# bwohlberg/sporco

Measured on AMD Instinct MI355X. Metric: ConvBPDN ADMM iterations/s, higher is better.
Workload: dtype f32; 1 GPU; admm.cbpdn.ConvBPDN 512x512 greyscale, K=64 8x8 filters, N=32 images per GPU, lambda=0.05, default options (AutoRho, stats every iteration); global_images=32, parallelism=image-shard x1

## Files before the change

sporco_amd/csrc/api_admm_run.inc:

```
    bool admm_run_supported(const sporco_amd_admm_params &p) const {
        return !cplx && std::is_same<T, float>::value && rows_ok && mr_ok(p) && (fused || fused_slabs) && !fused_mc &&
               !tail_mode && !(p.flags & (F_XRRS | F_GRADREG | F_KEEP_X | F_FEVAL_Y)) &&
               (!(p.flags & F_JOINT) || joint_rows_ok(p)) && p.lmbda >= 0.0 && p.rho > 0.0 &&
               !std::getenv("SPORCO_AMD_HOST_LOOP");
    }

    bool persist_ok(const sporco_amd_admm_params &p, const sporco_amd_admm_ctrl &c, bool vf,
                    bool has_reduce) const {
        const bool off = sw.persist >= 0 ? sw.persist != 1 : !hint_one_launch;
        return !off && vf && !has_reduce && fused && !fused_slabs && Ks == K && run_always_emit &&
               admm_persist_supported<T>(H, W, K) && !wl1.ptr && c.max_iter >= 3 &&
               !(p.flags & (F_NOBNDRY | F_AMS | F_JOINT)) && admm_persist_resident<T>(H, W, K, CN);
    }
    PersistIterArgs<T> persist_iter_args(const sporco_amd_admm_params &p, const T *vin, T *vout,
                                         double *prow, double *pcol) {
        PersistIterArgs<T> a;
        cx<T> *Xf = cv(SPORCO_AMD_VAR_XF);
        a.fwd.y = a.fwd.u = nullptr;
        a.fwd.v = vin;
        a.fwd.flags = p.flags;
        a.fwd.C = C;
        a.fwd.N = N;
        a.fwd.dH = p.dH;
        a.fwd.dW = p.dW;
// ... 69 lines not shown
        a.iter[p0] = persist_iter_args(p, v_prev, v_other, part_rows, part_f);
        a.iter[p0 ^ 1] = persist_iter_args(p, v_other, v_prev, pst_part_rows, pst_part_f);
        a.blk = static_cast<PersistIterArgs<T> *>(pst_blk);
        a.ctl_blk = pst_ctl;
        a.ctl = ctl_dev;
        a.rec = reinterpret_cast<AdmmRecord *>(rec_ring) + index0;
        a.index0 = index0;
        a.max_iter = max_iter - index0;
        a.bar = pst_bar;
        a.n_row_tiles = (int)nrow;
        a.n_col_tiles = (int)ncol;
        a.want_dfid = (p.flags & F_OBJ) ? 1 : 0;
        a.want_sums = want_sums ? 1 : 0;
        a.dfid_scale = 1.0 / ((double)H * W);
        SA_HIP(hipMemsetAsync(pst_bar, 0, sizeof(unsigned) * kPersistBarWords, st));
        {
            ProfScope ps(prof, PS_PERSIST);
            launch_admm_persist<T>(st, a, grid);
        }
        unsigned bar[16];
        SA_HIP(hipMemcpyAsync(bar, pst_bar, sizeof(bar), hipMemcpyDeviceToHost, st));
        sync();
        if (bar[2]) throw Error(SPORCO_AMD_EHIP, "one-launch solve: a grid barrier did not complete");
        xf_tiled = true;
        ++pst_runs;
        return (int)bar[3];
    }

    int64_t enqueue_iter_ctl(const sporco_amd_admm_params &p, const T *vin = nullptr,
                             T *vout = nullptr) {
        T *Y = vin ? nullptr : static_cast<T *>(vars[SPORCO_AMD_VAR_Y]);
        T *U = vin ? nullptr : static_cast<T *>(vars[SPORCO_AMD_VAR_U]);
        cx<T> *Xf = cv(SPORCO_AMD_VAR_XF);
        {
            RowsFwdArgs<T> ra;
            ra.y = Y;
            ra.u = U;
            ra.v = vin;
            ra.flags = p.flags;
            ra.C = C;
            ra.N = N;
            if (vin) {
                ra.wl1 = wl1;
                ra.dH = p.dH;
                ra.dW = p.dW;
                ra.ams_bits = ams_bits_of(p);
                ra.ams_k = Ku - 1;
            }
            ra.s2 = T(1);
            ra.t = Xf;
            ra.Ks = Ks;
            ra.twA = twRows;
            ra.H = H;
            ra.W = W;
            ra.CN = CN;
            ra.K = K;
            ra.P = P;
            ra.ctl = ctl_dev;
            ProfScope ps(prof, vin ? PS_ROWS_FWD_V : PS_ROWS_FWD);
            launch_rows_fwd<T>(st, ra);
        }
        {
            FusedColsArgs<T> fa;
            fa.t = Xf;
            fa.dft = dft;
            fa.sft = sft;
            fa.gramt = gramt;
            fa.twA = twA;
            fa.twB = twB;
            fa.rho = (T)p.rho;
            fa.H = H;
            fa.W = W;
            fa.CN = CN;
            fa.K = K;
            fa.partials = part_f;
            fa.Ks = Ks;
            fa.ctl = ctl_dev;
            if (cols_striped() && !fused_slabs) {
                fa.out_even = cols_out[0];
                fa.out_odd = cols_out[1];
            }
            ProfScope ps(prof, PS_FUSED_COLS);
            if (fused_slabs) {
                FusedSlabArgs<T> sa;
                sa.c = fa;
                sa.qpart = qpart;
                part_f_rows = (int)run_slab_cols(sa);
            } else {
                part_f_rows = (int)launch_fused_cols<T>(st, fa);
            }
            xf_tiled = true;
        }
        RowsPostArgs<T> pa;
        pa.twA = twRows;
        pa.t_next = nullptr;
        pa.t = Xf;
        if (cols_striped() && !fused_slabs) {
            pa.t = cols_out[0];
            pa.t_odd = cols_out[1];
        }
        pa.twW = planW.tw<T>();
        pa.y = Y;
        pa.u = U;
        pa.y_out = y_alt;
        pa.u_out = u_alt;
        pa.v_in = vin;
        pa.v_out = vout;
        pa.x = nullptr;
        pa.scale = T(1.0 / ((double)H * (double)W));
        pa.rlx = (T)p.rlx;
        pa.thr = T(0);
        pa.u_scale = T(1);
        pa.flags = p.flags;
// ... 204 lines not shown
        x_stale = true;
        x_invalid = p.flags & F_NO_X;
        prev_in_alt = !vf;
        return n;
    }

    void rows_inverse_to(T *Xout, const cx<T> *t_in = nullptr) {
        RowsProxArgs<T> ra;
        ra.t_in = t_in ? t_in : cv(SPORCO_AMD_VAR_XF);
        ra.Ks = t_in ? 0 : Ks;
        ra.t_out = nullptr;
        ra.x = Xout;
        ra.twA = twRows;
        ra.twW = planW.tw<T>();
        ra.scale = T(1.0 / ((double)H * (double)W));
        ra.thr = T(0);
        ra.flags = 0;
        ra.H = H;
        ra.W = W;
        ra.C = C;
        ra.N = N;
        ra.K = K;
        ra.dH = 1;
        ra.dW = 1;
        ra.P = P;
        ra.wl1 = Weight<T>();
        ra.partials = part_rows;
        ProfScope ps(prof, PS_FFT_C2R);
        launch_rows_inv_prox_fwd<T>(st, ra);
    }

    void launch_rows_fwd_on(const T *Yin, const T *Uin, T s2, const T *Vin = nullptr,
                            T thr_prev = T(0), uint32_t flags = 0, T thr21_prev = T(0),
                            const sporco_amd_admm_params *vp = nullptr, cx<T> *t_out = nullptr) {
        RowsFwdArgs<T> ra;
        if (Vin && vp) {
            ra.wl1 = wl1;
            ra.dH = vp->dH;
            ra.dW = vp->dW;
            ra.ams_bits = ams_bits_of(*vp);
            ra.ams_k = Ku - 1;
        }
        ra.y = Yin;
        ra.u = Uin;
        ra.v = Vin;
        ra.thr_prev = thr_prev;
        ra.thr21_prev = thr21_prev;
        ra.flags = flags;
        ra.C = C;
        ra.N = N;
        ra.s2 = s2;
        ra.t = t_out ? t_out : cv(SPORCO_AMD_VAR_XF);
        ra.Ks = Ks;
        ra.twA = twRows;
        ra.H = H;
        ra.W = W;
        ra.CN = CN;
        ra.K = K;
        ra.P = P;
        ProfScope ps(prof, Vin ? PS_ROWS_FWD_V : PS_ROWS_FWD);
        launch_rows_fwd<T>(st, ra);
    }
```

sporco_amd/csrc/api_setup.inc:

```
    void set_signal(const void *S) override {
        before_state_change();
        SA_HIP(hipMemcpyAsync(sreal, S, sizeof(T) * (int64_t)H * W * CNs, hipMemcpyHostToDevice, st));
        fwd2(sreal, nullptr, T(0), cv(SPORCO_AMD_VAR_SF), CNs);
        if (cplx_pair) pm_pair(cv(SPORCO_AMD_VAR_SF), cv(SPORCO_AMD_VAR_SF), 1, N, 1);
        refresh_fused_signal();
        sync();
        have_signal = true;
    }

    void set_signal_dev(const void *S_dev) override {
        before_state_change();
        SA_HIP(hipMemcpyAsync(sreal, S_dev, sizeof(T) * (int64_t)H * W * CNs,
                              hipMemcpyDeviceToDevice, st));
        fwd2(sreal, nullptr, T(0), cv(SPORCO_AMD_VAR_SF), CNs);
        if (cplx_pair) pm_pair(cv(SPORCO_AMD_VAR_SF), cv(SPORCO_AMD_VAR_SF), 1, N, 1);
        refresh_fused_signal();
        sync();
        have_signal = true;
    }

    void set_dict(const void *D, int dH, int dW) override {
        SA_REQUIRE(dH >= 1 && dW >= 1 && dH <= H && dW <= W,
                   "filter support must fit inside the signal");
        before_dict_change();
// ... 181 lines not shown
                materialize_x();
                prev_in_alt = keep;
                ProfScope ps(prof, PS_OTHER);
                launch_relax<T>(st, rv(SPORCO_AMD_VAR_X), y_alt, rv(SPORCO_AMD_VAR_AX),
                                (T)last_p.rlx, E);
            }
        }
        before_read(var);
        host_copy(var, dst, false);
        sync();
    }
    void *device_ptr(int var) override {
        before_read(var);
        return var_ptr(var);
    }

    void read_out(const double *out_dev, double *out_host) override {
        SA_HIP(hipMemcpyAsync(out_pinned, out_dev, sizeof(double) * kOutSlots, hipMemcpyDeviceToHost,
                              st));
        sync();
        std::memcpy(out_host, out_pinned, sizeof(double) * kOutSlots);
    }

    void require_single_channel_dict() const {
        if (Cd > 1)
            throw Error(SPORCO_AMD_EINVAL,
                        "multi-channel dictionaries are handled by the ADMM ConvBPDN calls only");
    }
    void require_ready() const {
        if (!have_dict || !have_signal)
            throw Error(SPORCO_AMD_ESTATE, "set_signal and set_dict must be called first");
    }

    bool run_fused_cols(const sporco_amd_admm_params &p, double *out_dev, bool striped = false) {
        if (fused_mc) {
            SA_REQUIRE(!(p.flags & (F_GRADREG | F_AMS | F_JOINT)),
                       "this solver variant needs a single-channel dictionary");
            if (!binv_valid || binv_rho != p.rho) {
                ProfScope ps(prof, PS_OTHER);
                launch_mc_binv<T>(st, dft_mc, bt_mc, npix, Cd, K, (T)p.rho);
                binv_valid = true;
                binv_rho = p.rho;
            }
            FusedMcArgs<T> ma;
            ma.t = cv(SPORCO_AMD_VAR_XF);
            ma.dft = dft_mc;
            ma.sft = sft_mc;
            ma.bt = bt_mc;
            ma.twA = twA;
            ma.twB = twB;
            ma.rho = (T)p.rho;
            ma.H = H;
            ma.W = W;
            ma.N = N;
            ma.K = K;
            ma.Cd = Cd;
            ma.partials = part_f;
            int64_t nt;
            {
                ProfScope ps(prof, PS_FUSED_COLS);
                nt = launch_fused_cols_mc<T>(st, ma);
            }
            part_f_rows = (int)nt;
            xf_tiled = true;
            if (out_dev && (p.flags & F_OBJ) && !(p.flags & F_FEVAL_Y)) {
                const int slots[1] = {SPORCO_AMD_OUT_DFID};
                const double scales[1] = {1.0 / ((double)H * W)};
// ... 37 lines not shown
        }
        int64_t ntiles;
        bool did_stripe = false;
        if (tail_ok) {
            if (!sft_eff) {
                SA_HIP(hipMalloc((void **)&sft_eff, sizeof(cx<T>) * npix * CN));
                SA_HIP(hipMalloc((void **)&coef_t, sizeof(cx<T>) * npix * CN));
            }
            const int Kt = K - 64;
            const int64_t nt = (int64_t)Wf * CN, tstride = (int64_t)H * Ks;
            cx<T> *tail = fa.t + 64;
            fa.Kv = 64;
            fa.Ks = Ks;
            fa.coef_out = coef_t;
            ProfScope ps(prof, PS_FUSED_COLS);
            fft_c2c<T>(st, planH, false, tail, tail, nt, Kt, tstride, Ks, tstride, Ks, T(1));
            launch_tail_inner<T>(st, fa, sft, sft_eff);
            fa.sft = sft_eff;
            ntiles = launch_fused_cols<T>(st, fa);
            launch_tail_update<T>(st, fa);
            fft_c2c<T>(st, planH, true, tail, tail, nt, Kt, tstride, Ks, tstride, Ks, T(1));
        } else if (fused_slabs) {
            FusedSlabArgs<T> sa;
            sa.c = fa;
            sa.qpart = qpart;
            ProfScope ps(prof, PS_FUSED_COLS);
            ntiles = run_slab_cols(sa);
            if (gradreg) ntiles *= (K + 63) / 64;
        } else {
            striped = striped && cols_striped() && !gradreg;
            if (striped) {
                fa.out_even = cols_out[0];
                fa.out_odd = cols_out[1];
            }
            ProfScope ps(prof, PS_FUSED_COLS);
            ntiles = launch_fused_cols<T>(st, fa);
            did_stripe = striped;
        }
        part_f_rows = (int)ntiles;
        xf_tiled = true;
        if (out_dev && (p.flags & F_OBJ) && !(p.flags & F_FEVAL_Y)) {
            const int slots[2] = {SPORCO_AMD_OUT_DFID, SPORCO_AMD_OUT_RGR};
            const double scales[2] = {1.0 / ((double)H * W), 1.0 / ((double)H * W)};
            const int nv = gradreg ? 2 : 1;
            finalize(part_f, (int)ntiles, nv, nv, slots, scales, out_dev);
        }
        return did_stripe;
    }

    void admm_iter_fused(const sporco_amd_admm_params &p, double *out_dev) {
        require_ready();
        if (gv_live) ensure_yu();
        const bool keep_x = p.flags & F_KEEP_X;
        const bool nn = p.flags & F_NONNEG, jn = p.flags & F_JOINT;
        if (v_live && (!vform_ok(p) || !vform_same_opts(p))) ensure_yu();
        const bool vf = vform_ok(p) && (v_live || touch_epoch == fused_epoch);
        T *vin = vf && v_live ? v_cur : nullptr;
        if (!keep_x && !y_alt) alloc_alt_pair();
        T *Y = vin ? nullptr : rv(SPORCO_AMD_VAR_Y), *U = vin ? nullptr : rv(SPORCO_AMD_VAR_U);
        cx<T> *Xf = cv(SPORCO_AMD_VAR_XF);
        T *vout = vf ? (vin == y_alt ? u_alt : y_alt) : nullptr;
        if (!(t_ready && p.u_scale == 1.0)) {
            if (vin) launch_rows_fwd_on(nullptr, nullptr, (T)p.u_scale, vin, v_thr, p.flags, v_thr21, &p);
            else launch_rows_fwd_on(Y, U, (T)p.u_scale);
        }
        t_ready = false;
        const bool striped = run_fused_cols(p, nullptr, !keep_x);
        stable_run = p.u_scale == 1.0 ? stable_run + 1 : 0;
        const bool emit = stable_run >= 2 && !sw.no_speculation;
        RowsPostArgs<T> pa;
        pa.twA = twRows;
        pa.t_next = emit ? Xf : nullptr;
        pa.t = Xf;
        if (striped) {
            pa.t = cols_out[0];
            pa.t_odd = cols_out[1];
        }
        pa.twW = planW.tw<T>();
        pa.y = Y;
        pa.u = U;
        pa.y_out = keep_x ? Y : y_alt;
        pa.u_out = keep_x ? U : u_alt;
        pa.v_in = vin;
        pa.v_out = vout;
        pa.thr_prev = v_thr;
        pa.thr21_prev = v_thr21;
        pa.x = keep_x ? rv(SPORCO_AMD_VAR_X) : nullptr;
        pa.scale = T(1.0 / ((double)H * (double)W));
        pa.rlx = (T)p.rlx;
        pa.thr = (T)(p.lmbda / p.rho);
        pa.thr21 = (T)(p.mu / p.rho);
        pa.u_scale = (T)p.u_scale;
        pa.flags = p.flags;
        pa.H = H;
        pa.W = W;
        pa.C = C;
        pa.N = N;
        pa.K = K;
        pa.dH = p.dH;
        pa.dW = p.dW;
// ... 60 lines not shown
```

sporco_amd/csrc/csc_api.hip:

```cpp
#include "csc_impl.h"

#include <chrono>
#include <string>

namespace sporco_amd {

thread_local std::string g_last_error;
std::atomic<int64_t> g_xfer[4];
const char *kProfNames[PS_COUNT] = {"fft_r2c_rows",     "fft_c2c_cols_fwd", "sm_solve",
                                           "fft_c2c_cols_inv", "fft_c2r_rows",     "admm_post",
                                           "fused_cols_sm",    "rows_fwd",         "rows_inv_post",
                                           "rows_inv_post_emit",
                                           "rows_fwd_v",       "rows_inv_post_v",  "rows_inv_post_v_emit",
                                           "pgm_grad_ifft",    "pgm_rows_prox",    "pgm_fft_momentum",
                                           "finalize",         "pgm_elementwise",  "other",
                                           "admm_persist_run",
                                    "setcoef_rows",     "setcoef_cols",     "ccmod_grad_tiled",
                                    "fft_c2r_vpost",    "fft_c2r_vpost_emit",
                                    "inhib_update"};

struct Switches {
    bool unfused, old_rows, no_pad, no_vform, no_speculation, no_cols_sm, md_generic, cns_generic, cg_host,
        placement_off, placement_force;
    int persist;
    int cols_sm_force_slab;
    static bool set(const char *name) { return std::getenv(name) != nullptr; }
    static Switches read() {
        Switches s;
        s.unfused = set("SPORCO_AMD_UNFUSED");
        s.old_rows = set("SPORCO_AMD_OLD_ROWS");
        s.no_pad = set("SPORCO_AMD_NO_PAD");
        s.no_vform = set("SPORCO_AMD_NO_VFORM");
        s.no_speculation = set("SPORCO_AMD_NO_SPECULATION");
        s.no_cols_sm = set("SPORCO_AMD_NO_COLS_SM");
        s.md_generic = set("SPORCO_AMD_MD_GENERIC");
        s.cns_generic = set("SPORCO_AMD_CNS_GENERIC");
        s.cg_host = set("SPORCO_AMD_CG_HOST");
        const char *e = std::getenv("SPORCO_AMD_PLACEMENT");
        s.placement_off = e && e[0] == '0';
        s.placement_force = e && e[0] == 'f';
        e = std::getenv("SPORCO_AMD_PERSIST");
        s.persist = e ? (e[0] == '1' ? 1 : 0) : -1;
        e = std::getenv("SPORCO_AMD_COLS_SM_FORCE_SLAB");
        s.cols_sm_force_slab = e ? std::atoi(e) : 0;
        return s;
    }
};

template <typename T> struct Csc : CscBase {
    const Switches sw = Switches::read();
    sporco_amd_dims dm;
    int device;
    hipStream_t st = nullptr;
    bool own_stream = false;
    int H, W, Wf, C, N, K, CN;
    int Ku;
    int Cd = 1, Cs, CNs;
    cx<T> *ism_gam = nullptr, *ism_del = nullptr, *ism_mm = nullptr;
    bool fused_mc = false;
    cx<T> *dft_mc = nullptr, *sft_mc = nullptr;
    T *bt_mc = nullptr;
    bool binv_valid = false;
    double binv_rho = 0.0;
    cx<T> *cns_f = nullptr;
    static constexpr int kTailMax = 8;
    int Ks = 0;
    int64_t EFt = 0;
    bool tail_mode = false;
    cx<T> *sft_eff = nullptr, *coef_t = nullptr;
    uint32_t *ams_bits = nullptr;
    bool ams_bits_valid = false;
    T *cns_m = nullptr, *cns_yold = nullptr;
    bool cns_active = false;
// ... 227 lines not shown
    }
    void big_alloc_fresh(void **p, size_t bytes) {
        if (bytes >= ((size_t)64 << 20)) {
            const size_t al = (size_t)kAllocAlignMb << 20;
            void *base = nullptr;
            SA_HIP(hipMalloc(&base, bytes + al));
            const uintptr_t b = reinterpret_cast<uintptr_t>(base);
            *p = reinterpret_cast<void *>((b + al - 1) / al * al);
            skew_reg.emplace_back(*p, base);
            return;
        }
        SA_HIP(hipMalloc(p, bytes));
    }
    void big_free(void *p) {
        if (!p) return;
        for (auto &e : skew_reg)
            if (e.first == p) {
                (void)hipFree(e.second);
                e.first = nullptr;
                return;
            }
        (void)hipFree(p);
    }

    ~Csc() override {
        (void)hipSetDevice(device);
        (void)hipStreamSynchronize(st);
        place_release_spares();
        inhib_release();
        big_free(gemit);
        if (part_vpost) (void)hipFree(part_vpost);
        big_free(cols_out[0]);
        big_free(cols_out[1]);
        for (hipEvent_t e : place_ev)
            if (e) (void)hipEventDestroy(e);
        for (auto &v : vars) big_free(v);
        big_free(y_alt);
        big_free(u_alt);
        big_free(work);
        y_alt = u_alt = nullptr;
        work = nullptr;
        for (void *p : {(void *)pst_part_rows, (void *)pst_part_f, pst_blk, (void *)pst_ctl, (void *)pst_bar,
                        (void *)cns_w, (void *)cns_sft, (void *)flt_h, (void *)flt_w,
                        (void *)zf_ch, (void *)zfv_buf, (void *)md_sft, (void *)md_coef, (void *)pgm_rx[0], (void *)pgm_rx[1]})
            if (p) (void)hipFree(p);
        for (void *p : {(void *)dft, (void *)sft, (void *)gramt, (void *)part_f, (void *)twA, (void *)twB,
                        (void *)twRows, (void *)part_rows, (void *)y_alt, (void *)u_alt, (void *)part_pgm, (void *)part_pgm2, (void *)ccmod_r, (void *)pgm_ey, (void *)gpart,
                        (void *)qpart, (void *)coop_flags, (void *)ghh, (void *)ghw, (void *)wg, (void *)g1t, (void *)ism_gam, (void *)ism_del, (void *)ism_mm, (void *)dft_mc, (void *)sft_mc, (void *)bt_mc, (void *)cns_f, (void *)cns_m, (void *)sft_eff, (void *)coef_t, (void *)ams_bits, (void *)gramz_t,
                        (void *)cns_yold, (void *)md_s, (void *)dism_gam, (void *)dism_del, (void *)dism_mm,
                        (void *)dwork, (void *)pcn_stats, (void *)work, (void *)innerb, (void *)gram, (void *)dpad, (void *)sreal,
                        (void *)wl1_buf, (void *)wl21_buf, (void *)wams_buf, (void *)wdat_buf, (void *)part_a, (void *)part_b, (void *)part_cs, (void *)df_im, (void *)pgm_es[0], (void *)pgm_es[1], (void *)pgm_es[2], (void *)pgm_es[3],
                        (void *)out_dev_own})
            if (p) (void)hipFree(p);
        if (out_pinned) (void)hipHostFree(out_pinned);
        if (coop_err) (void)hipHostFree(coop_err);
        if (rec_ring) (void)hipHostFree(rec_ring);
        if (cg_pin) (void)hipHostFree((void *)cg_pin);
        if (cg_dev) (void)hipFree(cg_dev);
        if (ctl_dev) (void)hipFree(ctl_dev);
        planW.destroy();
        planH.destroy();
        if (depth > 1) planD.destroy();
        if (own_stream) (void)hipStreamDestroy(st);
    }

    int64_t KD() const { return (int64_t)Cd * K; }
// ... 46 lines not shown
    void sync() override {
        SA_HIP(hipStreamSynchronize(st));
        if (coop_err && *coop_err) {
            *coop_err = 0;
            throw Error(SPORCO_AMD_EHIP, "cooperating slab workgroups: a partner's partial sums never "
                                         "arrived; the iterates of this handle are invalid");
        }
    }
    bool pgm_fused_ok() const {
        return rows_ok && (cols256 || mr) && (fused || (fused_slabs && !tail_mode && !mr));
    }
    bool hint_vform = false, hint_one_launch = false;
    bool cplx_pair = false;
    void set_hint(int what, int value) override {
        if (what == SPORCO_AMD_HINT_KEEP_VFORM) hint_vform = value != 0;
        else if (what == SPORCO_AMD_HINT_ONE_LAUNCH) hint_one_launch = value != 0;
        else if (what == SPORCO_AMD_MODE_COMPLEX_PAIR) {
            SA_REQUIRE(Cd == 2 && Cs == 2, "complex pair mode: a handle with two channels (real, imaginary)");
            SA_REQUIRE(!have_signal && !zf_ch, "complex pair mode is set before the signal and the coefficient maps");
            cplx_pair = value != 0;
        } else if (what == SPORCO_AMD_VOLUME_FILTER_DEPTH) {
            SA_REQUIRE(depth > 1 && value >= 1 && value <= depth, "filter depth: a volume handle, 1 <= value <= depth");
            SA_REQUIRE(!flt_h, "volume handle: one filter support (no multi-scale dictionary)");
            vol_dD = value;
        } else throw Error(SPORCO_AMD_EINVAL, "unknown hint");
    }
    void pm_pair(const cx<T> *src, cx<T> *dst, int mid, int inner, int mode) {
        ProfScope ps(prof, PS_OTHER);
        launch_pm_butterfly<T>(st, src, dst, npix, mid, inner, W, mode);
    }
    std::string placement() override { return placement_report(); }
    cx<T> *cols_out[2] = {nullptr, nullptr};
    bool cols_striped() const { return cols_out[0] != nullptr; }
    void alloc_cols_out() {
        if (cols_out[0] || !std::is_same<T, float>::value || !fused || fused_slabs || tail_mode || Ks != K || !rows_ok || mr)
            return;
        const size_t plane = sizeof(cx<T>) * (size_t)CN * H * K;
        const size_t be = plane * (size_t)((Wf + 1) / 2), bo = plane * (size_t)(Wf / 2);
        if (!placement_on(be)) return;
        void *p0 = nullptr;
        big_alloc(&p0, be);
        cols_out[0] = static_cast<cx<T> *>(p0);
        cols_out[1] = static_cast<cx<T> *>(place_alloc(bo, {{p0, be}}, "cols_out_odd"));
    }
    void alloc_alt_pair() {
        if (y_alt) return;
        (void)var_ptr(SPORCO_AMD_VAR_XF);
        place_var(SPORCO_AMD_VAR_XF, {SPORCO_AMD_VAR_Y, SPORCO_AMD_VAR_U}, "T");
        void *t = vars[SPORCO_AMD_VAR_XF];
        const size_t tb = var_alloc_bytes(SPORCO_AMD_VAR_XF), nb = sizeof(T) * (size_t)E;
        y_alt = static_cast<T *>(place_alloc(nb, {{t, tb}}, "V0"));
        u_alt = static_cast<T *>(place_alloc(nb, {{t, tb}}, "V1"));
        place_var(SPORCO_AMD_VAR_Y, {SPORCO_AMD_VAR_XF}, "Y");
        place_var(SPORCO_AMD_VAR_U, {SPORCO_AMD_VAR_XF}, "U");
        alloc_cols_out();
        place_release_spares();
    }
    int query(int what) override {
        if (what == SPORCO_AMD_QUERY_FUSED_COLS) return (fused || fused_slabs || fused_mc) ? 1 : 0;
        if (what == SPORCO_AMD_QUERY_FUSED_ROWS) return rows_ok ? 1 : 0;
        if (what == SPORCO_AMD_QUERY_FUSED_PGM) return pgm_fused_ok() ? 1 : 0;
        if (what == SPORCO_AMD_QUERY_DEVICE_FILTERS) return K;
        if (what == SPORCO_AMD_QUERY_VFORM_LIVE) return (v_live || gv_live) ? 1 : 0;
        if (what == SPORCO_AMD_QUERY_PERSIST_RUNS) return pst_runs;
        if (what == SPORCO_AMD_QUERY_CCMOD_GROUPS) return ccmod_group_count();
        throw Error(SPORCO_AMD_EINVAL, "unknown query");
    }

#include "api_placement.inc"
#include "api_transforms.inc"
#include "api_setup.inc"
#include "api_admm_run.inc"
#include "api_admm.inc"
#include "api_pgm.inc"
#include "api_dictupdate.inc"
#include "api_consensus.inc"
// ... 13 lines not shown
```

sporco_amd/csrc/csc_fused.h:

```cpp
#pragma once

#include "common.h"
#include "csc_kernels.h"

namespace sporco_amd {

constexpr int kColsStaggerGroups = 4, kColsStaggerSleeps = 2;

template <typename E>
void launch_permute_ab(hipStream_t st, const E *in, E *out, int64_t A, int64_t B, int64_t C,
                       int64_t in_stride = 0, int64_t out_stride = 0);

template <typename T> struct FusedColsArgs {
    cx<T> *t;
    const cx<T> *dft;
    const cx<T> *sft;
    const T *gramt;
    const cx<T> *twA;
    const cx<T> *twB;
    T rho;
    int H, W, CN, K;
    double *partials;
    int Kv = 0;
    cx<T> *coef_out = nullptr;
    int Ks = 0;
    int per_tile = 0;
    int stagger_groups = 1, stagger_sleeps = 0;
    const AdmmCtl *ctl = nullptr;
    cx<T> *out_even = nullptr, *out_odd = nullptr;
    const T *g1t = nullptr;
    T *g1t_out = nullptr;
    const T *ghh = nullptr, *ghw = nullptr, *wg = nullptr;
    T mu = T(0);
};
template <typename T>
void launch_tail_inner(hipStream_t st, const FusedColsArgs<T> &a, const cx<T> *sft, cx<T> *sft_eff);
template <typename T> void launch_tail_update(hipStream_t st, const FusedColsArgs<T> &a);
template <typename T> void launch_gram_rows(hipStream_t st, const cx<T> *z, T *out, int64_t nrows, int K);
template <typename T> void launch_grad_g1(hipStream_t st, const FusedColsArgs<T> &a);

template <typename T> struct FusedSlabArgs {
    FusedColsArgs<T> c;
    cx<T> *qpart;
    unsigned *coop_flags = nullptr;
    unsigned coop_seq = 0;
    int *coop_err = nullptr;
    const cx<T> *pgm_yf = nullptr;
    T pgm_inv_L = T(0);
    cx<T> *pgm_ey = nullptr;
};
template <typename T> int64_t launch_cols_slab_coop(hipStream_t st, const FusedSlabArgs<T> &a);
template <typename T> int64_t launch_pgm_grad_slabs(hipStream_t st, const FusedSlabArgs<T> &a);
template <typename T> bool fused_slabs_supported(int H, int K);

template <typename T> struct FusedMcArgs {
    cx<T> *t;
    const cx<T> *dft;
    const cx<T> *sft;
    const T *bt;
    const cx<T> *twA, *twB;
    T rho;
    int H, W, N, K, Cd;
// ... 18 lines not shown
```

sporco_amd/csrc/csc_fused_body.inc:

```

    constexpr int H = N1 * NW;
    constexpr bool MR = mr_length(N1);
    constexpr int J = MR ? (N1 > NW ? 2 : 1) : N1 / NW;
    constexpr int LBW = ilog2(NW);
    static_assert(!MR || (NW == 16 && LP == 1), "mixed-radix heights: 16 waves, one line per group");
    constexpr int FP = LP * NW, Q = J / LP;
    static_assert(J % LP == 0, "lines per group must divide the lines per thread");
    static_assert(FP * NW * 64 <= kExchUnitsMax, "exchange group too large");
    const int tid = threadIdx.x;
    const int k = tid & 63;
    const int w = sa_readfirstlane(tid >> 6);
    const int K = (KC && !KRT) ? KC : ((KRT && a.Ks) ? a.Ks : a.K);
    const bool kv = KC == 64 ? true : k < K;
    const int xcd = blockIdx.x & 7;
    f2 *LA = dyn_lds<f2>();
    f2 *LB = LA;
    double *scratch = reinterpret_cast<double *>(LA + FP * NW * 64);
    const cf zero = mk<float>(0.f, 0.f);
    const int cvoff = k == 0 ? 0 : (int)0x80000000;
    const int ko = (w * K + k) * (int)sizeof(cf);
    int token = 0;
    if constexpr (AOFF >= 0) {
        if (a.ctl && a.ctl->stop) return;
        if constexpr (PERSIST) {
            const int ph = (int)(blockIdx.x >> 3) % a.stagger_groups;
            for (int i = 0; i < ph * a.stagger_sleeps; ++i) __builtin_amdgcn_s_sleep(127);
        }
    }
    for (int slot = blockIdx.x >> 3;; slot += gridDim.x >> 3) {
    SA_ARGS_PTR_T(FusedColsArgs<float>) ap;
    if constexpr (AOFF >= 0) ap = sa_args_reload<PERSIST, AOFF>(a);
    else ap = sa_opaque_sptr(afix);
    const int Wf = ap->W / 2 + 1, CN = ap->CN;
    if (slot >= ((Wf + 7) / 8) * CN) break;
    const int wf = (slot / CN) * 8 + xcd;
    if (wf >= Wf) break;
    const int tile = wf * CN + slot % CN;
    const AdmmCtl *ctl = ap->ctl;
    const float rho = ctl ? ctl->rho_f : ap->rho;
    const float *GH = ap->ghh + w;
    const cf *twA = ap->twA + w * N1;
    const cf *twB = ap->twB + w * (J * NW);
    const BufRsrc Tb = make_rsrc(ap->t + (int64_t)tile * H * K, (uint32_t)(H * K * sizeof(cf)));
    const int dsel = PER_TILE ? tile : wf;
    const BufRsrc Db = make_rsrc(ap->dft + (int64_t)dsel * H * K, (uint32_t)(H * K * sizeof(cf)));
    cf *const coef_out = KRT ? ap->coef_out : nullptr;
    const BufRsrc Cb = make_rsrc(coef_out ? coef_out + (int64_t)tile * H : nullptr,
                                 coef_out ? (uint32_t)(H * sizeof(cf)) : 0u);
    const cf *S = ap->sft + (int64_t)tile * H + w;
    const float *G = (GRAD ? ap->g1t : ap->gramt) + (int64_t)dsel * H + w;

    unsigned long long ts[16] = {0};
    SA_TS(0)
    cf v[N1];
#pragma unroll
    for (int h1 = 0; h1 < N1; ++h1)
        v[h1] = (kv && DBG != 2 && DBG != 4) ? buf_load_cf_x<(AOFF < 0)>(Tb, ko, NW * h1 * K * (int)sizeof(cf))
                                 : mk<float>((float)(k + h1), (float)(w - h1));
    if constexpr (DBG != 1) {
    dif1<N1, false>(v, 0);
    reg_fence<N1>(v, 0, token);
#pragma unroll
    for (int i = 1; i < N1; ++i) {
        cf tw;
        if constexpr (KC == 64 && !GRAD) sa_uload2(reinterpret_cast<const float *>(twA + i), tw.re, tw.im);
        else tw = twA[i];
        v[i] = cmul(v[i], tw);
    }
    reg_fence<N1>(v, 0, token);
    }
    SA_TS(1)

    float obj = 0.f;
    if constexpr (DBG != 1) {
    float ak = 0.f, bk = 0.f, gw = 0.f, rg = 0.f;
    if constexpr (GRAD) {
// ... 173 lines not shown
```

sporco_amd/csrc/csc_rows.h:

```cpp
#pragma once

#include "common.h"
#include "csc_fused.h"
#include "csc_kernels.h"

namespace sporco_amd {

template <typename T> struct RowsFwdArgs {
    const T *y, *u;
    T s2;
    cx<T> *t;
    const cx<T> *twA;
    int H, W, CN, K;
    int64_t P;
    const T *v = nullptr;
    T thr_prev = T(0);
    uint32_t flags = 0;
    T thr21_prev = T(0);
    int C = 1, N = 0;
    Weight<T> wl1;
    int dH = 1, dW = 1;
    const uint32_t *ams_bits = nullptr;
    int ams_k = -1;
    int y_bcast = 0;
    int Ks = 0;
    const AdmmCtl *ctl = nullptr;
    int persist = 0;
    int stagger_groups = 1, stagger_sleeps = 0;
};

template <typename T> struct RowsPostArgs {
    const cx<T> *t;
    const cx<T> *t_odd = nullptr;
    const cx<T> *twW;
    const cx<T> *twA;
    cx<T> *t_next;
    int emit_u = 0;
    const T *y, *u;
    T *y_out, *u_out;
    T *x;
    const T *v_in = nullptr;
    T *v_out = nullptr;
    T thr_prev = T(0);
    T thr21_prev = T(0);
// ... 69 lines not shown
```

sporco_amd/csrc/csc_rows_body.inc:

```
#include "csc_rows.h"

#include <cmath>
#include <cstdlib>

#include "csc_ctl_dev.h"
#include "csc_fused_body.h"
#include "regfft.h"

namespace sporco_amd {

namespace {

using namespace regfft;

struct alignas(16) cf2 {
    cf a, b;
};

constexpr int kN1 = 32;
constexpr size_t rows_lds_bytes(int NW) {
    return sizeof(f2) * 16 * NW * 64 + sizeof(double) * 8 * 16;
}

template <int N1, int NW> constexpr int spectral_waves() { return regfft::mr_length(N1) ? (N1 + 1) / 2 : NW; }
// ... 12 lines not shown

__host__ __device__ constexpr bool first_half4(int k1) {
    return k1 < 4 || k1 == 8 || (k1 >= 13 && k1 <= 19) || k1 == 24 || k1 > 28;
}
__host__ __device__ constexpr int group_of(int N1, int NW, int k1) {
    if (NW == 4) return first_half4(k1) ? 0 : 1;
    return NW == 16 ? (k1 >= (N1 + 1) / 2 ? 1 : 0) : ((k1 < 8 || k1 == 16 || k1 > 24) ? 0 : 1);
}
__host__ __device__ constexpr int kl_of(int N1, int NW, int k1) {
    if (NW == 4) {
        int r = 0;
        for (int o = 0; o < k1; ++o) r += first_half4(o) == first_half4(k1) ? 1 : 0;
        return r;
    }
    if (NW == 16) return k1 >= (N1 + 1) / 2 ? k1 - (N1 + 1) / 2 : k1;
    if (group_of(N1, NW, k1) == 0) return k1 < 8 ? k1 : (k1 == 16 ? 8 : k1 - 16);
    return k1 < 16 ? k1 - 8 : k1 - 9;
}

__device__ __forceinline__ float soft1(float v, float thr) {
    float m = fabsf(v) - thr;
    m = m > 0.f ? m : 0.f;
    return __builtin_copysignf(m, v);
}
__device__ __forceinline__ float soft1_pos(float v, float thr) { return v - sa_med3(v, -thr, thr); }
template <int MODE> __device__ __forceinline__ float soft1_m(float v, float thr) {
    if constexpr (MODE == 1) return soft1(v, thr);
    else return soft1_pos(v, thr);
}

template <int NW, bool COH = false, int N1 = kN1>
__device__ __forceinline__ void spatial_to_spectral(cf (&v)[N1], const cf *twA, cf *t, int CN, int H,
                                                    int K, int cn, int k, int h, bool pv, int w,
                                                    int lane, f2 *L, int &token) {
    constexpr int J = spectral_lines<N1, NW>(), NA = spectral_waves<N1, NW>();
    constexpr int NG = 2;
    constexpr int LPG = J / NG;
    constexpr int LBW = ilog2(NW);
    const bool act = NA >= NW || w < NA;
    dif1<N1, false>(v, 0);
#pragma unroll
    for (int i = 1; i < N1; ++i) {
        cf tw;
        sa_uload2(reinterpret_cast<const float *>(twA + w * N1 + i), tw.re, tw.im);
        v[i] = cmul(v[i], tw);
    }
    reg_fence<N1>(v, 0, token);

    cf z[J * NW];
    static_for<NG>([&](auto gc) {
        constexpr int g = decltype(gc)::value;
#pragma unroll
        for (int k1 = 0; k1 < N1; ++k1) {
            if (group_of(N1, NW, k1) != g) continue;
            const cf x = v[pos1<N1>(k1)];
            f2 t;
            t.x = x.re;
            t.y = x.im;
            L[(kl_of(N1, NW, k1) * NW + w) * 64 + lane] = t;
        }
        __syncthreads();
        if (act && (g == 0 || second_line<N1>(w))) {
#pragma unroll
            for (int jl = 0; jl < LPG; ++jl) {
                const int j = g * LPG + jl;
                const int kl = kl_of(N1, NW, line_of<N1, NW>(w, j));
#pragma unroll
                for (int n2 = 0; n2 < NW; ++n2) {
                    const f2 t = L[(kl * NW + n2) * 64 + lane];
                    z[NW * j + n2] = mk<float>(t.x, t.y);
                }
            }
        } else if (act) {
#pragma unroll
            for (int i = 0; i < LPG * NW; ++i) z[NW * g * LPG + i] = mk<float>(0.f, 0.f);
        }
        if (g + 1 < NG) __syncthreads();
    });
    if (!act) return;

#pragma unroll
    for (int j = 0; j < J; ++j) dif<NW, false>(z, NW * j);

    const int64_t tline = (int64_t)CN * H * K;
    cf *Tl = t + (int64_t)cn * H * K + (int64_t)h * K + k;
    auto store_unit = [&](int f, cf zf, cf zp) {
        cf2 ab;
        ab.a = mk<float>(0.5f * (zf.re + zp.re), 0.5f * (zf.im - zp.im));
        ab.b = mk<float>(0.5f * (zf.im + zp.im), 0.5f * (zp.re - zf.re));
        if (pv) {
            const float q[4] = {ab.a.re, ab.a.im, ab.b.re, ab.b.im};
            if constexpr (COH) sa_coh_store4(reinterpret_cast<float *>(Tl + (int64_t)f * tline), q);
            else sa_stream_store4(reinterpret_cast<float *>(Tl + (int64_t)f * tline), q);
        }
    };
#pragma unroll
    for (int pr = 0; pr < J / 2; ++pr) {
        const int ja = 2 * pr, jb = 2 * pr + 1;
        const int k1a = line_of<N1, NW>(w, ja), k1b = line_of<N1, NW>(w, jb);
        if (pr == 0 && w == 0) {
#pragma unroll
            for (int k2 = 0; k2 <= NW / 2; ++k2) {
                const cf zf = z[NW * ja + brev(k2 % NW, LBW)];
                const cf zp = z[NW * ja + brev((NW - k2) % NW, LBW)];
                store_unit(N1 * k2, zf, zp);
            }
            if constexpr ((N1 & 1) == 0) {
#pragma unroll
            for (int k2 = 0; k2 < NW / 2; ++k2) {
                const cf zf = z[NW * jb + brev(k2, LBW)];
                const cf zp = z[NW * jb + brev(NW - 1 - k2, LBW)];
                store_unit(N1 / 2 + N1 * k2, zf, zp);
            }
            }
        } else {
#pragma unroll
            for (int k2 = 0; k2 < NW / 2; ++k2) {
                store_unit(k1a + N1 * k2, z[NW * ja + brev(k2, LBW)],
                           z[NW * jb + brev(NW - 1 - k2, LBW)]);
                store_unit(k1b + N1 * k2, z[NW * jb + brev(k2, LBW)],
                           z[NW * ja + brev(NW - 1 - k2, LBW)]);
            }
        }
    }
}

// ... 214 lines not shown
                    float q0 = y0 * y0, q1 = y1 * y1;
                    sum_over_rows2(q0, q1);
                    float f0 = sa_fma(-thr21_p, sa_rsq(q0), 1.f);
                    float f1 = sa_fma(-thr21_p, sa_rsq(q1), 1.f);
                    f0 = f0 > 0.f ? f0 : 0.f;
                    f1 = f1 > 0.f ? f1 : 0.f;
                    y0 = f0 * y0;
                    y1 = f1 * y1;
                }
                y0 = sa_med3(y0, am_e[0] ? -__builtin_inff() : nn_lo, __builtin_inff());
                y1 = sa_med3(y1, am_e[1] ? -__builtin_inff() : nn_lo, __builtin_inff());
                if constexpr (GENERAL) {
                    const int n1 = half * HB + i;
                    const float keep = (hkill || NW * n1 + w >= x0kill) ? 0.f : 1.f;
                    const float mkeep = ((mbits >> n1) & 1u) ? 0.f : 1.f;
                    y0 *= am_e[0] ? mkeep : keep;
                    y1 *= am_e[1] ? mkeep : keep;
                }
                yv[i] = mk<float>(y0, y1);
                uv[i] = mk<float>(vv.re - y0, vv.im - y1);
            }
        }
#pragma unroll
        for (int i = 0; i < HB; ++i) {
#pragma clang fp contract(off)
            if (half * HB + i >= N1) continue;
            v[half * HB + i] = mk<float>(sa_fma(-s2, uv[i].re, yv[i].re), sa_fma(-s2, uv[i].im, yv[i].im));
        }
        if constexpr ((N1 & 1) == 0) reg_fence<HB>(v, half * HB, token);
        else if (half == 0) reg_fence<HB>(v, 0, token);
        else reg_fence<N1 - HB>(v, HB, token);
    }
    spatial_to_spectral<NW, COH, N1>(v, a->twA, a->t, a->CN, a->H, a->Ks ? a->Ks : a->K, cn, k, h, pv, w, lane, L,
                                     token);
}

template <typename A, typename F>
__device__ __forceinline__ void rows_tile_loop(const A &a_in, int tiles_x, int tiles_y, F &&tile_fn) {
    const int64_t ntiles = (int64_t)tiles_x * tiles_y;
    if (a_in.persist) {
        const int ph = (int)(blockIdx.x % (unsigned)a_in.stagger_groups);
        for (int i = 0; i < ph * a_in.stagger_sleeps; ++i) __builtin_amdgcn_s_sleep(127);
    }
    for (int64_t t = blockIdx.x; t < ntiles; t += gridDim.x) {
        tile_fn(sa_args_reload(a_in), (int)(t % tiles_x), (int)(t / tiles_x));
        __syncthreads();
    }
}

template <int NW, bool BCAST, bool VFORM = false, bool JOINT = false, int MODE = 0, int N1 = kN1>
__global__ void __launch_bounds__(NW * 64) rows_fwd_kernel(const RowsFwdArgs<float> a_in) {
    if (a_in.ctl && (a_in.ctl->stop | a_in.ctl->skip_fwd)) return;
    const int tiles_x = JOINT ? a_in.N * (a_in.K >> 5) : (int)((a_in.P + 127) / 128);
    rows_tile_loop(a_in, tiles_x, a_in.H,
                   [](auto a, int bx, int h) { rows_fwd_tile<NW, BCAST, VFORM, JOINT, MODE, false, N1>(a, bx, h); });
}

constexpr int batch_of(int n, int want) {
    int b = 1;
    for (int d = 1; d <= want; ++d)
        if (n % d == 0) b = d;
    return b;
}
template <int NW, bool WRITE_X, int MODE, bool EMIT_T, bool JOINT, int SF, bool COH = false, int N1 = kN1,
          typename AP>
__device__ __forceinline__ void rows_inv_post_tile(AP a, int bx, int h, int tiles_x) {
    constexpr bool GENERAL = MODE != 0;
// ... 543 lines not shown
        return 1;
    } else {
        return 2;
    }
}

template <int NW, int N1, bool EMIT, int MODE, bool JOINT>
void rows_post_variant(dim3 grid, hipStream_t st, const RowsPostArgs<float> &a) {
    if (a.v_out) {
        SA_REQUIRE(!a.x, "the V form has no X output");
        if (a.v_in) rows_launch<NW, &rows_inv_post_kernel<NW, false, MODE, EMIT, JOINT, 2, N1>>(grid, st, a);
        else rows_launch<NW, &rows_inv_post_kernel<NW, false, MODE, EMIT, JOINT, 1, N1>>(grid, st, a);
        return;
    }
    SA_REQUIRE(!a.v_in, "a V-form input needs a V-form output");
    if constexpr (!JOINT) {
        if (a.x) return rows_launch<NW, &rows_inv_post_kernel<NW, true, MODE, EMIT, false, 0, N1>>(grid, st, a);
    }
    rows_launch<NW, &rows_inv_post_kernel<NW, false, MODE, EMIT, JOINT, 0, N1>>(grid, st, a);
}
template <int NW, int N1, bool EMIT> void rows_post_emit(dim3 grid, hipStream_t st, RowsPostArgs<float> &a) {
    if (a.flags & F_JOINT) return rows_post_variant<NW, N1, EMIT, 0, true>(grid, st, a);
    const int mode = rows_mode<N1>(a);
    if (mode == 0) rows_post_variant<NW, N1, EMIT, 0, false>(grid, st, a);
    else if (mode == 1) rows_post_variant<NW, N1, EMIT, 1, false>(grid, st, a);
    else if constexpr (!mr_length(N1)) rows_post_variant<NW, N1, EMIT, 2, false>(grid, st, a);
}

}

template <int NW, int N1> void rows_fwd_launch(hipStream_t st, RowsFwdArgs<float> a) {
    constexpr bool MR = regfft::mr_length(N1);
    SA_REQUIRE(!(MR && a.y_bcast), "mixed-radix widths: no broadcast form");
    if (a.v && (a.flags & F_JOINT)) {
        SA_REQUIRE(rows_joint_supported<float>(a.W, a.C, a.K) && a.C * a.N == a.CN && !a.wl1.ptr && !a.ams_bits &&
                       !(a.flags & F_NOBNDRY),
                   "configuration not handled by the joint row pass");
        const dim3 jgrid = rows_grid(a, NW, (int64_t)a.N * (a.K / 32), a.H, 0);
        return rows_launch<NW, &rows_fwd_kernel<NW, false, true, true, 0, N1>>(jgrid, st, a);
    }
    const dim3 grid = rows_grid(a, NW, ceil_div(a.P, 128), a.H, 0);
    if (!a.v) {
        if constexpr (!MR) {
            if (a.y_bcast) return rows_launch<NW, &rows_fwd_kernel<NW, true, false, false, 0, N1>>(grid, st, a);
        }
        return rows_launch<NW, &rows_fwd_kernel<NW, false, false, false, 0, N1>>(grid, st, a);
    }
    const int mode = rows_mode<N1>(a);
    SA_REQUIRE(mode == 0 || a.C * a.N == a.CN, "the derivation needs the channel / image split");
    if (mode == 0) rows_launch<NW, &rows_fwd_kernel<NW, false, true, false, 0, N1>>(grid, st, a);
    else if (mode == 1) rows_launch<NW, &rows_fwd_kernel<NW, false, true, false, 1, N1>>(grid, st, a);
    else if constexpr (!MR) rows_launch<NW, &rows_fwd_kernel<NW, false, true, false, 2, N1>>(grid, st, a);
}

template <int NW, int N1> int64_t rows_inv_post_launch(hipStream_t st, RowsPostArgs<float> a) {
    SA_REQUIRE(!(regfft::mr_length(N1) && a.t_odd), "mixed-radix widths: no striped spectrum");
    const bool joint = a.flags & F_JOINT;
    if (joint) {
        SA_REQUIRE(!a.v_in || a.v_out, "a V-form input needs a V-form output");
        SA_REQUIRE(rows_joint_supported<float>(a.W, a.C, a.K) && !a.wl1.ptr && !a.ams_bits &&
                       !(a.flags & F_NOBNDRY) && !a.x,
                   "configuration not handled by the joint row epilogue");
    }
    const int64_t tx = joint ? (int64_t)a.N * (a.K / 32) : ceil_div(a.P, 128);
    const dim3 grid = rows_grid(a, NW, tx, a.H, a.t_next != nullptr);
    if (a.t_next) rows_post_emit<NW, N1, true>(grid, st, a);
// ... 24 lines not shown
```

Measured before the change: 390.2 iterations/s (512x512, K=64, N=32 per GPU; summed over GPUs).

## Stripe row-FFT spectrum output into even/odd buffers with separate placement

After: 390.1 iterations/s (512x512, K=64, N=32 per GPU; summed over GPUs) (median of 3 runs). About the same (-0.0%).

```diff
diff --git a/sporco_amd/csrc/api_admm_run.inc b/sporco_amd/csrc/api_admm_run.inc
--- a/sporco_amd/csrc/api_admm_run.inc
+++ b/sporco_amd/csrc/api_admm_run.inc
@@ -125,6 +125,7 @@
         T *Y = vin ? nullptr : static_cast<T *>(vars[SPORCO_AMD_VAR_Y]);
         T *U = vin ? nullptr : static_cast<T *>(vars[SPORCO_AMD_VAR_U]);
         cx<T> *Xf = cv(SPORCO_AMD_VAR_XF);
+        const bool tstripe = tfwd_striped(p);
         {
             RowsFwdArgs<T> ra;
             ra.y = Y;
@@ -142,6 +143,7 @@
             }
             ra.s2 = T(1);
             ra.t = Xf;
+            if (tstripe) ra.t_odd = tfwd_odd;
             ra.Ks = Ks;
             ra.twA = twRows;
             ra.H = H;
@@ -172,6 +174,7 @@
             if (cols_striped() && !fused_slabs) {
                 fa.out_even = cols_out[0];
                 fa.out_odd = cols_out[1];
+                if (tstripe) fa.t_odd = tfwd_odd;
             }
             ProfScope ps(prof, PS_FUSED_COLS);
             if (fused_slabs) {
@@ -442,7 +445,8 @@
 
     void launch_rows_fwd_on(const T *Yin, const T *Uin, T s2, const T *Vin = nullptr,
                             T thr_prev = T(0), uint32_t flags = 0, T thr21_prev = T(0),
-                            const sporco_amd_admm_params *vp = nullptr, cx<T> *t_out = nullptr) {
+                            const sporco_amd_admm_params *vp = nullptr, cx<T> *t_out = nullptr,
+                            bool stripe = false) {
         RowsFwdArgs<T> ra;
         if (Vin && vp) {
             ra.wl1 = wl1;
@@ -461,6 +465,7 @@
         ra.N = N;
         ra.s2 = s2;
         ra.t = t_out ? t_out : cv(SPORCO_AMD_VAR_XF);
+        if (stripe) ra.t_odd = tfwd_odd;
         ra.Ks = Ks;
         ra.twA = twRows;
         ra.H = H;
diff --git a/sporco_amd/csrc/api_setup.inc b/sporco_amd/csrc/api_setup.inc
--- a/sporco_amd/csrc/api_setup.inc
+++ b/sporco_amd/csrc/api_setup.inc
@@ -237,7 +237,9 @@
             throw Error(SPORCO_AMD_ESTATE, "set_signal and set_dict must be called first");
     }
 
-    bool run_fused_cols(const sporco_amd_admm_params &p, double *out_dev, bool striped = false) {
+    bool run_fused_cols(const sporco_amd_admm_params &p, double *out_dev, bool striped = false,
+                        bool in_striped = false) {
+        SA_REQUIRE(!in_striped || (striped && tfwd_striped(p)), "striped row spectrum without a striped column pass");
         if (fused_mc) {
             SA_REQUIRE(!(p.flags & (F_GRADREG | F_AMS | F_JOINT)),
                        "this solver variant needs a single-channel dictionary");
@@ -341,6 +343,7 @@
             if (striped) {
                 fa.out_even = cols_out[0];
                 fa.out_odd = cols_out[1];
+                if (in_striped) fa.t_odd = tfwd_odd;
             }
             ProfScope ps(prof, PS_FUSED_COLS);
             ntiles = launch_fused_cols<T>(st, fa);
@@ -369,12 +372,13 @@
         T *Y = vin ? nullptr : rv(SPORCO_AMD_VAR_Y), *U = vin ? nullptr : rv(SPORCO_AMD_VAR_U);
         cx<T> *Xf = cv(SPORCO_AMD_VAR_XF);
         T *vout = vf ? (vin == y_alt ? u_alt : y_alt) : nullptr;
+        const bool tstripe = !keep_x && !(t_ready && p.u_scale == 1.0) && tfwd_striped(p);
         if (!(t_ready && p.u_scale == 1.0)) {
-            if (vin) launch_rows_fwd_on(nullptr, nullptr, (T)p.u_scale, vin, v_thr, p.flags, v_thr21, &p);
-            else launch_rows_fwd_on(Y, U, (T)p.u_scale);
+            if (vin) launch_rows_fwd_on(nullptr, nullptr, (T)p.u_scale, vin, v_thr, p.flags, v_thr21, &p, nullptr, tstripe);
+            else launch_rows_fwd_on(Y, U, (T)p.u_scale, nullptr, T(0), 0, T(0), nullptr, nullptr, tstripe);
         }
         t_ready = false;
-        const bool striped = run_fused_cols(p, nullptr, !keep_x);
+        const bool striped = run_fused_cols(p, nullptr, !keep_x, tstripe);
         stable_run = p.u_scale == 1.0 ? stable_run + 1 : 0;
         const bool emit = stable_run >= 2 && !sw.no_speculation;
         RowsPostArgs<T> pa;
diff --git a/sporco_amd/csrc/csc_api.hip b/sporco_amd/csrc/csc_api.hip
--- a/sporco_amd/csrc/csc_api.hip
+++ b/sporco_amd/csrc/csc_api.hip
@@ -21,7 +21,7 @@
 
 struct Switches {
     bool unfused, old_rows, no_pad, no_vform, no_speculation, no_cols_sm, md_generic, cns_generic, cg_host,
-        placement_off, placement_force;
+        placement_off, placement_force, no_stripe_tfwd;
     int persist;
     int cols_sm_force_slab;
     static bool set(const char *name) { return std::getenv(name) != nullptr; }
@@ -39,6 +39,8 @@
         const char *e = std::getenv("SPORCO_AMD_PLACEMENT");
         s.placement_off = e && e[0] == '0';
         s.placement_force = e && e[0] == 'f';
+        e = std::getenv("SPORCO_AMD_STRIPE_TFWD");
+        s.no_stripe_tfwd = e && e[0] == '0';
         e = std::getenv("SPORCO_AMD_PERSIST");
         s.persist = e ? (e[0] == '1' ? 1 : 0) : -1;
         e = std::getenv("SPORCO_AMD_COLS_SM_FORCE_SLAB");
@@ -332,6 +334,7 @@
         if (part_vpost) (void)hipFree(part_vpost);
         big_free(cols_out[0]);
         big_free(cols_out[1]);
+        big_free(tfwd_odd);
         for (hipEvent_t e : place_ev)
             if (e) (void)hipEventDestroy(e);
         for (auto &v : vars) big_free(v);
@@ -444,6 +447,11 @@
     std::string placement() override { return placement_report(); }
     cx<T> *cols_out[2] = {nullptr, nullptr};
     bool cols_striped() const { return cols_out[0] != nullptr; }
+    cx<T> *tfwd_odd = nullptr;
+    bool tfwd_striped(const sporco_amd_admm_params &p) const {
+        return tfwd_odd && cols_striped() && !fused_mc && !fused_slabs && !tail_mode &&
+               !(p.flags & (F_GRADREG | F_JOINT));
+    }
     void alloc_cols_out() {
         if (cols_out[0] || !std::is_same<T, float>::value || !fused || fused_slabs || tail_mode || Ks != K || !rows_ok || mr)
             return;
@@ -454,6 +462,8 @@
         big_alloc(&p0, be);
         cols_out[0] = static_cast<cx<T> *>(p0);
         cols_out[1] = static_cast<cx<T> *>(place_alloc(bo, {{p0, be}}, "cols_out_odd"));
+        if (!sw.no_stripe_tfwd)
+            tfwd_odd = static_cast<cx<T> *>(place_alloc(bo, {{vars[SPORCO_AMD_VAR_XF], var_alloc_bytes(SPORCO_AMD_VAR_XF)}}, "rows_fwd_t_odd"));
     }
     void alloc_alt_pair() {
         if (y_alt) return;
diff --git a/sporco_amd/csrc/csc_fused.h b/sporco_amd/csrc/csc_fused.h
--- a/sporco_amd/csrc/csc_fused.h
+++ b/sporco_amd/csrc/csc_fused.h
@@ -28,6 +28,7 @@
     int stagger_groups = 1, stagger_sleeps = 0;
     const AdmmCtl *ctl = nullptr;
     cx<T> *out_even = nullptr, *out_odd = nullptr;
+    const cx<T> *t_odd = nullptr;
     const T *g1t = nullptr;
     T *g1t_out = nullptr;
     const T *ghh = nullptr, *ghw = nullptr, *wg = nullptr;
diff --git a/sporco_amd/csrc/csc_fused_body.inc b/sporco_amd/csrc/csc_fused_body.inc
--- a/sporco_amd/csrc/csc_fused_body.inc
+++ b/sporco_amd/csrc/csc_fused_body.inc
@@ -20,8 +20,10 @@
     const int cvoff = k == 0 ? 0 : (int)0x80000000;
     const int ko = (w * K + k) * (int)sizeof(cf);
     int token = 0;
+    int fwd_in = 1;
     if constexpr (AOFF >= 0) {
         if (a.ctl && a.ctl->stop) return;
+        if (a.ctl) fwd_in = a.ctl->skip_fwd ? 0 : 1;
         if constexpr (PERSIST) {
             const int ph = (int)(blockIdx.x >> 3) % a.stagger_groups;
             for (int i = 0; i < ph * a.stagger_sleeps; ++i) __builtin_amdgcn_s_sleep(127);
@@ -41,7 +43,12 @@
     const float *GH = ap->ghh + w;
     const cf *twA = ap->twA + w * N1;
     const cf *twB = ap->twB + w * (J * NW);
-    const BufRsrc Tb = make_rsrc(ap->t + (int64_t)tile * H * K, (uint32_t)(H * K * sizeof(cf)));
+    const cf *tin = ap->t + (int64_t)tile * H * K;
+    if constexpr (AOFF >= 0 && !MR) {
+        if (ap->t_odd && (wf & 1) && fwd_in)
+            tin = ap->t_odd + ((int64_t)(wf >> 1) * CN + slot % CN) * H * K;
+    }
+    const BufRsrc Tb = make_rsrc(tin, (uint32_t)(H * K * sizeof(cf)));
     const int dsel = PER_TILE ? tile : wf;
     const BufRsrc Db = make_rsrc(ap->dft + (int64_t)dsel * H * K, (uint32_t)(H * K * sizeof(cf)));
     cf *const coef_out = KRT ? ap->coef_out : nullptr;
diff --git a/sporco_amd/csrc/csc_rows.h b/sporco_amd/csrc/csc_rows.h
--- a/sporco_amd/csrc/csc_rows.h
+++ b/sporco_amd/csrc/csc_rows.h
@@ -10,6 +10,7 @@
     const T *y, *u;
     T s2;
     cx<T> *t;
+    cx<T> *t_odd = nullptr;
     const cx<T> *twA;
     int H, W, CN, K;
     int64_t P;
diff --git a/sporco_amd/csrc/csc_rows_body.inc b/sporco_amd/csrc/csc_rows_body.inc
--- a/sporco_amd/csrc/csc_rows_body.inc
+++ b/sporco_amd/csrc/csc_rows_body.inc
@@ -68,7 +68,7 @@
 template <int NW, bool COH = false, int N1 = kN1>
 __device__ __forceinline__ void spatial_to_spectral(cf (&v)[N1], const cf *twA, cf *t, int CN, int H,
                                                     int K, int cn, int k, int h, bool pv, int w,
-                                                    int lane, f2 *L, int &token) {
+                                                    int lane, f2 *L, int &token, cf *t_odd = nullptr) {
     constexpr int J = spectral_lines<N1, NW>(), NA = spectral_waves<N1, NW>();
     constexpr int NG = 2;
     constexpr int LPG = J / NG;
@@ -120,14 +120,16 @@
 
     const int64_t tline = (int64_t)CN * H * K;
     cf *Tl = t + (int64_t)cn * H * K + (int64_t)h * K + k;
+    const int64_t odd_delta = t_odd ? t_odd - t : 0;
     auto store_unit = [&](int f, cf zf, cf zp) {
         cf2 ab;
         ab.a = mk<float>(0.5f * (zf.re + zp.re), 0.5f * (zf.im - zp.im));
         ab.b = mk<float>(0.5f * (zf.im + zp.im), 0.5f * (zp.re - zf.re));
         if (pv) {
             const float q[4] = {ab.a.re, ab.a.im, ab.b.re, ab.b.im};
-            if constexpr (COH) sa_coh_store4(reinterpret_cast<float *>(Tl + (int64_t)f * tline), q);
-            else sa_stream_store4(reinterpret_cast<float *>(Tl + (int64_t)f * tline), q);
+            const int64_t poff = (t_odd && (f & 1)) ? (int64_t)(f >> 1) * tline + odd_delta : (int64_t)f * tline;
+            if constexpr (COH) sa_coh_store4(reinterpret_cast<float *>(Tl + poff), q);
+            else sa_stream_store4(reinterpret_cast<float *>(Tl + poff), q);
         }
     };
 #pragma unroll
@@ -408,7 +410,7 @@
         else reg_fence<N1 - HB>(v, HB, token);
     }
     spatial_to_spectral<NW, COH, N1>(v, a->twA, a->t, a->CN, a->H, a->Ks ? a->Ks : a->K, cn, k, h, pv, w, lane, L,
-                                     token);
+                                     token, a->t_odd);
 }
 
 template <typename A, typename F>
@@ -1018,6 +1020,7 @@
 template <int NW, int N1> void rows_fwd_launch(hipStream_t st, RowsFwdArgs<float> a) {
     constexpr bool MR = regfft::mr_length(N1);
     SA_REQUIRE(!(MR && a.y_bcast), "mixed-radix widths: no broadcast form");
+    SA_REQUIRE(!a.t_odd || (!MR && (!a.Ks || a.Ks == a.K) && !(a.flags & F_JOINT)), "striped spectrum: power-of-two widths, rows of K filters, not joint");
     if (a.v && (a.flags & F_JOINT)) {
         SA_REQUIRE(rows_joint_supported<float>(a.W, a.C, a.K) && a.C * a.N == a.CN && !a.wl1.ptr && !a.ams_bits &&
                        !(a.flags & F_NOBNDRY),
```
